# BloodAxe/segmentation-networks-benchmark

Hardware: AMD Instinct MI355X
Metric: images/sec/GPU (fwd+bwd) ZF_UNET 224x224 bs=32; 1/2/4/8-GPU scaling (higher is better)
Workload: dtype bf16; 1 GPU; ZF_UNET 224x224 bf16 bs=32/GPU, bce_dice, SGD lr 1e-3, Dropout2d 0.2, train step torch_train.py:180-190 (configs[1]); global_batch=32, parallelism=dp1

## Files before the change

segmentation-networks-benchmark_amd/csrc/common.h:

```cpp
#pragma once
#include <hip/hip_runtime.h>
#include <hip/hip_ext.h>
#include <stdint.h>
#include <stdio.h>
#include <string.h>

#include "../../include/segnb_hip.h"

typedef __attribute__((ext_vector_type(8))) __bf16 bf16x8_t;
typedef __attribute__((ext_vector_type(16))) float f32x16_t;

struct bf16_t {
    unsigned short bits;
};

void segnb_set_error(const char* fmt, ...);

#define SEGNB_CHECK_ARG(cond, msg)                                   \
    do {                                                             \
        if (!(cond)) {                                               \
            segnb_set_error("%s: bad argument: %s", __func__, msg);  \
            return SEGNB_E_BADARG;                                   \
        }                                                            \
    } while (0)
// ... 73 lines not shown
void segnb_plan_refuse(const char* why);
#define SEGNB_PLAN_REFUSE(why)                                         \
    SegnbPlanScope plan_scope__;                                       \
    if (plan_scope__.top && g_segnb_census_on) segnb_census(__func__); \
    if (plan_scope__.top && segnb_plan_recording()) segnb_plan_refuse(why)

int segnb_num_cus();
int segnb_knob_fprop_dma();
int segnb_knob_fprop_dma_cfg();
int segnb_knob_fprop_dma_dbg();
int segnb_knob_fprop_nostats();
int segnb_knob_rw_store_waves();
int segnb_knob_bnreduce_fused();
int segnb_knob_fprop_deepk();
int segnb_knob_fprop_thin();
enum segnb_try_outcome {
    SEGNB_TRY_DECLINED = 0,
    SEGNB_TRY_LAUNCHED,
    SEGNB_TRY_DELIVERED,
};
inline int segnb_try_launched(segnb_try_outcome* did, int rc) {
    if (rc == 0) *did = SEGNB_TRY_LAUNCHED;
    return rc;
}
int segnb_fprop_thin_try(segnb_try_outcome* did, const segnb_conv_geom* g, const void* in, const void* wpacked, void* out,
                         hipStream_t stream, const segnb_bn_reduce_epilogue* bn);
int segnb_fprop_thin_ok(const segnb_conv_geom* g);
int segnb_knob_fprop_upd();
int segnb_knob_fprop_drop();
int segnb_knob_fprop_mask();
int segnb_fprop_dma_actmask_ok(const segnb_conv_geom* g);
int segnb_fprop_roll_actmask_ok(const segnb_conv_geom* g);
int segnb_knob_fprop_mf16();
int segnb_knob_fprop_rw();
int segnb_knob_fprop_ksplit();
float* segnb_head_scratch(size_t bytes, hipStream_t stream);
void segnb_head_bwd_finish(const float* part, int gx, int gy, int K, int C, int CT, float* dw, float* db, hipStream_t stream);
int segnb_knob_pack_blocks();
int segnb_knob_fprop_roll();
int segnb_knob_wg_cu_pct();
int segnb_knob_conv_cus();
int segnb_fprop_dma_read_stamps(unsigned long long* host_dst);
int segnb_fprop_s1_try(segnb_try_outcome* did, const segnb_conv_geom* g, const void* in, const void* wpacked, const float* bias, int bias_n,
                       void* out, double* stats, hipStream_t stream, const float* drop = nullptr, int ld_drop = 0, int stats_ld = 0);
int segnb_fprop_dma_try(segnb_try_outcome* did, const segnb_conv_geom* g, const void* in, unsigned in_bytes, const void* wpacked,
                        unsigned w_bytes, const float* bias, int bias_n, void* out, double* stats,
                        hipStream_t stream, const segnb_act_epilogue* ep = nullptr, const segnb_upcat_src* uc = nullptr,
                        const segnb_bn_reduce_epilogue* bn = nullptr);
int segnb_fprop_rw_try(segnb_try_outcome* did, const segnb_conv_geom* g, const void* in, unsigned in_bytes, const void* wpacked,
                       unsigned w_bytes, const float* bias, int bias_n, void* out, double* stats,
                       hipStream_t stream, const segnb_bn_reduce_epilogue* bn = nullptr,
                       const segnb_act_epilogue* ep = nullptr, const segnb_upcat_src* uc = nullptr,
                       const segnb_upcat_src* upsum = nullptr);
int segnb_fprop_roll_try(segnb_try_outcome* did, const segnb_conv_geom* g, const void* in, unsigned in_bytes, const void* wpacked,
                         unsigned w_bytes, const float* bias, int bias_n, void* out, double* stats, hipStream_t stream,
                         const segnb_bn_reduce_epilogue* bn = nullptr, const segnb_operand_tf* tf = nullptr,
                         const segnb_upcat_src* uc = nullptr);
int segnb_fprop_c8_try(segnb_try_outcome* did, const segnb_conv_geom* g, const void* in, const void* wpacked, const float* bias, int bias_n,
                       void* out, double* stats, hipStream_t stream, const segnb_act_epilogue* ep = nullptr);
struct segnb_wgrad_bnapply {
    const void* g;
    int ld_g;
    const void* y;
    int ld_y;
    const float* coef;
    const float* bcoef;
// ... 106 lines not shown
```

segmentation-networks-benchmark_amd/csrc/runtime.hip:

```cpp
#include <stdarg.h>
#include <stdlib.h>

#include "common.h"

static thread_local char g_err[512] = "";

void segnb_set_error(const char* fmt, ...) {
    va_list ap;
    va_start(ap, fmt);
    vsnprintf(g_err, sizeof(g_err), fmt, ap);
    va_end(ap);
}

int segnb_num_cus() {
    static int cus = 0;
    if (cus > 0) return cus;
    int dev = 0;
    hipDeviceProp_t prop;
    if (hipGetDevice(&dev) != hipSuccess || hipGetDeviceProperties(&prop, dev) != hipSuccess) return 256;
    cus = prop.multiProcessorCount > 0 ? prop.multiProcessorCount : 256;
    return cus;
}

extern "C" const char* segnb_last_error(void) { return g_err; }
// ... 232 lines not shown
}
static int g_pack_blocks = 0;
int segnb_knob_pack_blocks() { return g_pack_blocks; }

static int g_wgrad_roll = 0;
int segnb_knob_wgrad_roll() { return g_wgrad_roll; }
static int g_wgrad_c8roll = 1;
int segnb_knob_wgrad_c8roll() { return g_wgrad_c8roll; }
static int g_conv_cu_pct = 100;
int segnb_knob_conv_cus() {
    const int n = segnb_num_cus() * g_conv_cu_pct / 100;
    return n < 1 ? 1 : n;
}
static int g_wg_cu_pct = 0;
int segnb_knob_wg_cu_pct() { return g_wg_cu_pct; }
static int g_fprop_deepk = -2;
int segnb_knob_fprop_deepk() {
    if (g_fprop_deepk == -2) {
        const char* e = getenv("SEGNB_FPROP_DEEPK");
        g_fprop_deepk = (e != nullptr && e[0] == '0') ? 0 : 1;
    }
    return g_fprop_deepk;
}
static int g_fprop_thin = 1;
int segnb_knob_fprop_thin() { return g_fprop_thin; }
static int g_fprop_mf16 = -2;
int segnb_knob_fprop_mf16() {
    if (g_fprop_mf16 == -2) {
        const char* e = getenv("SEGNB_FPROP_MF16");
        g_fprop_mf16 = (e != nullptr && e[0] == '0') ? 0 : 1;
    }
    return g_fprop_mf16;
}
static int g_fprop_upd = -2;
int segnb_knob_fprop_upd() {
    if (g_fprop_upd == -2) {
        const char* e = getenv("SEGNB_FPROP_UPD");
        g_fprop_upd = (e != nullptr && e[0] == '0') ? 0 : 1;
    }
    return g_fprop_upd;
}
static int g_fprop_mask = -2;
int segnb_knob_fprop_mask() {
    if (g_fprop_mask == -2) {
        const char* e = getenv("SEGNB_FPROP_MASK");
        g_fprop_mask = (e != nullptr && e[0] == '0') ? 0 : 1;
    }
    return g_fprop_mask;
}
static int g_fprop_drop = -2;
int segnb_knob_fprop_drop() {
    if (g_fprop_drop == -2) {
        const char* e = getenv("SEGNB_FPROP_DROP");
        g_fprop_drop = (e != nullptr && e[0] == '0') ? 0 : 1;
    }
    return g_fprop_drop;
}
static int g_fprop_nostats = 1;
int segnb_knob_fprop_nostats() { return g_fprop_nostats; }
static int g_rw_store_waves = 4;
int segnb_knob_rw_store_waves() { return g_rw_store_waves; }
static int g_bnreduce_fused = -2;
int segnb_knob_bnreduce_fused() {
    if (g_bnreduce_fused == -2) {
        const char* e = getenv("SEGNB_BNREDUCE_FUSED");
        g_bnreduce_fused = (e != nullptr && e[0] == '0') ? 0 : 1;
// ... 80 lines not shown
    }
    if (strcmp(key, "fprop_drop") == 0) {
        g_fprop_drop = value ? 1 : 0;
        return 0;
    }
    if (strcmp(key, "fprop_mask") == 0) {
        g_fprop_mask = value ? 1 : 0;
        return 0;
    }
    if (strcmp(key, "fprop_nostats") == 0) {
        g_fprop_nostats = value ? 1 : 0;
        return 0;
    }
    if (strcmp(key, "rw_store_waves") == 0) {
        g_rw_store_waves = value == 2 ? 2 : (value == 8 ? 8 : 4);
        return 0;
    }
    if (strcmp(key, "bnreduce_fused") == 0) {
        g_bnreduce_fused = value ? 1 : 0;
        return 0;
    }
    if (strcmp(key, "fprop_deepk") == 0) {
        g_fprop_deepk = value ? 1 : 0;
        return 0;
    }
    if (strcmp(key, "fprop_thin") == 0) {
        g_fprop_thin = value ? 1 : 0;
        return 0;
    }
    if (strcmp(key, "fprop_mf16") == 0) {
        g_fprop_mf16 = value ? 1 : 0;
        return 0;
    }
    if (strcmp(key, "call_census") == 0) {
        g_segnb_census_on = value ? 1 : 0;
        return 0;
    }
    if (strcmp(key, "fprop_ksplit") == 0) {
        g_fprop_ksplit = value < 0 ? 0 : value;
        return 0;
    }
    if (strcmp(key, "fprop_dma_dbg") == 0) {
        g_fprop_dma_dbg = value;
        return 0;
    }
    segnb_set_error("segnb_tune: unknown key '%s'", key);
    return SEGNB_E_BADARG;
}

extern "C" int segnb_debug_stamps(unsigned long long* host_dst) {
    SEGNB_CHECK_ARG(host_dst != nullptr, "NULL destination");
    return segnb_fprop_dma_read_stamps(host_dst);
}
```

segmentation-networks-benchmark_amd/csrc/wgrad_s1.hip:

```cpp
#include "common.h"

#include <cstdlib>
#include <type_traits>

namespace {

typedef __attribute__((ext_vector_type(4))) __bf16 bf16x4_t;
typedef __attribute__((address_space(3))) bf16x4_t* lds_bf16x4_ptr;

__device__ __forceinline__ bf16x8_t tr_frag(const unsigned char* p, int row4_bytes) {
    const bf16x4_t lo = __builtin_amdgcn_ds_read_tr16_b64_v4bf16((lds_bf16x4_ptr)(p));
    const bf16x4_t hi = __builtin_amdgcn_ds_read_tr16_b64_v4bf16((lds_bf16x4_ptr)(p + row4_bytes));
    return __builtin_shufflevector(lo, hi, 0, 1, 2, 3, 4, 5, 6, 7);
}

typedef __attribute__((address_space(3))) unsigned char* lds_u8_ptr;
__device__ __forceinline__ unsigned lds_addr(const void* p) { return (unsigned)(uintptr_t)(lds_u8_ptr)p; }

#define SEGNB_TR_READ2(lo, hi, addr, off0, off1)                                           \
    asm volatile("ds_read_b64_tr_b16 %0, %2 offset:%3\n\tds_read_b64_tr_b16 %1, %2 offset:%4" \
                 : "=&v"(lo), "=&v"(hi)                                                    \
                 : "v"(addr), "n"(off0), "n"(off1))
#define SEGNB_MFMA(acc, af, bf) \
    asm volatile("v_mfma_f32_32x32x16_bf16 %0, %1, %2, %0" : "+a"(acc) : "v"(af), "v"(bf))
#define SEGNB_MFMA_V(acc, af, bf) \
    asm volatile("v_mfma_f32_32x32x16_bf16 %0, %1, %2, %0" : "+v"(acc) : "v"(af), "v"(bf))
#define SEGNB_WAIT_LGKM(n) asm volatile("s_waitcnt lgkmcnt(%0)" ::"n"(n))

#ifndef SEGNB_WG_TS
#define SEGNB_WG_TS 1
#endif
#ifndef SEGNB_WG_WS_DB
#define SEGNB_WG_WS_DB 0
#endif
#ifndef SEGNB_WG_PACE
#define SEGNB_WG_PACE 0
#endif
#ifndef SEGNB_WG_TALL
#define SEGNB_WG_TALL 1
#endif
#ifndef SEGNB_WG_EXP
#define SEGNB_WG_EXP 0
#endif

struct WgS1Args {
    const bf16_t* x;
    const bf16_t* dy;
    float* dwp;
    int N, H, W;
    int Hi, Wi;
    int Ci, Co, ld_x, ld_dy;
    int dhmin, dwmin;
    int dh[9], dw[9];
    int HB, WB, IT;
    int TCI_TILES;
// ... 15 lines not shown
__device__ __forceinline__ void wg_tap(f32x16_t (&acc)[9], const bf16x4_t (&fa)[2], bf16x4_t (&fbc)[9][2],
                                       bf16x4_t (&fbn)[9][2], const unsigned (&vb)[9]) {
    SEGNB_WAIT_LGKM(WAITN);
    const bf16x8_t af = __builtin_shufflevector(fa[0], fa[1], 0, 1, 2, 3, 4, 5, 6, 7);
    const bf16x8_t bf = __builtin_shufflevector(fbc[T][0], fbc[T][1], 0, 1, 2, 3, 4, 5, 6, 7);
    SEGNB_MFMA(acc[T], af, bf);
    if constexpr (MORE) SEGNB_TR_READ2(fbn[T][0], fbn[T][1], vb[T], OB, OB + 4 * SXB);
}

template <int S0, int SPW, int KSPLIT, int SEGS, int WT, int XC, int SX, int SY, int MID, typename F>
__device__ __forceinline__ void wg_slabs(f32x16_t (&acc)[9], bf16x4_t (&fa)[2][2], bf16x4_t (&fb)[2][9][2],
                                         unsigned va, const unsigned (&vb)[9], F& mid) {
    if constexpr (S0 < SPW) {
        if constexpr (S0 == MID) mid();
        constexpr int cur = S0 & 1, nxt = cur ^ 1;
        constexpr bool more = S0 + 1 < SPW;
        constexpr int sn = (S0 + 1) * KSPLIT;
        constexpr int oa = ((sn / SEGS) * WT + (sn % SEGS) * 16) * SY;
        constexpr int ob = ((sn / SEGS) * XC + (sn % SEGS) * 16) * SX;
        if constexpr (more) SEGNB_TR_READ2(fa[nxt][0], fa[nxt][1], va, oa, oa + 4 * SY);
        wg_tap<0, 15, more, ob, SX>(acc, fa[cur], fb[cur], fb[nxt], vb);
        wg_tap<1, more ? 15 : 14, more, ob, SX>(acc, fa[cur], fb[cur], fb[nxt], vb);
        wg_tap<2, more ? 15 : 12, more, ob, SX>(acc, fa[cur], fb[cur], fb[nxt], vb);
        wg_tap<3, more ? 15 : 10, more, ob, SX>(acc, fa[cur], fb[cur], fb[nxt], vb);
        wg_tap<4, more ? 15 : 8, more, ob, SX>(acc, fa[cur], fb[cur], fb[nxt], vb);
        wg_tap<5, more ? 15 : 6, more, ob, SX>(acc, fa[cur], fb[cur], fb[nxt], vb);
        wg_tap<6, more ? 15 : 4, more, ob, SX>(acc, fa[cur], fb[cur], fb[nxt], vb);
        wg_tap<7, more ? 15 : 2, more, ob, SX>(acc, fa[cur], fb[cur], fb[nxt], vb);
        wg_tap<8, more ? 15 : 0, more, ob, SX>(acc, fa[cur], fb[cur], fb[nxt], vb);
        wg_slabs<S0 + 1, SPW, KSPLIT, SEGS, WT, XC, SX, SY, MID>(acc, fa, fb, va, vb, mid);
    }
}

constexpr int ts_c(int G, int u) { return (u + G) & 1; }
constexpr int ts_b(int G, int u) { return (u + G) >> 1; }
constexpr int ts_fa(int G, int c) { return c == G ? 0 : 2; }
constexpr int ts_fb(int b) { return b == 0 ? 1 : b + 2; }
constexpr int ts_k(int G, int u) {
    const int ka = ts_fa(G, ts_c(G, u)), kb = ts_fb(ts_b(G, u));
    return ka > kb ? ka : kb;
}
constexpr int ts_wait(int G, int u, bool more) {
    const int w = (6 - ts_k(G, u)) * 2 + (more ? 2 * (u < 7 ? u : 7) : 0);
    return w > 15 ? 15 : w;
}

template <int G, int J, int OA, int OB, int SX, int SY>
__device__ __forceinline__ void ts_request(bf16x4_t (&fan)[2][2], bf16x4_t (&fbn)[5][2], unsigned va,
                                           const unsigned (&vb)[5]) {
    if constexpr (J == 0) {
        SEGNB_TR_READ2(fan[G][0], fan[G][1], va, OA + 64 * G, OA + 64 * G + 4 * SY);
    } else if constexpr (J == 2) {
        SEGNB_TR_READ2(fan[1 - G][0], fan[1 - G][1], va, OA + 64 * (1 - G), OA + 64 * (1 - G) + 4 * SY);
    } else {
        constexpr int B = J == 1 ? 0 : J - 2;
        SEGNB_TR_READ2(fbn[B][0], fbn[B][1], vb[B], OB, OB + 4 * SX);
    }
}

template <int G, int U, bool MORE, int OA, int OB, int SX, int SY>
__device__ __forceinline__ void ts_units(f32x16_t (&acc)[9], bf16x4_t (&fac)[2][2], bf16x4_t (&fbc)[5][2],
                                         bf16x4_t (&fan)[2][2], bf16x4_t (&fbn)[5][2], unsigned va,
                                         const unsigned (&vb)[5]) {
    if constexpr (U < 9) {
        constexpr int C = ts_c(G, U), B = ts_b(G, U);
        SEGNB_WAIT_LGKM(ts_wait(G, U, MORE));
        const bf16x8_t af = __builtin_shufflevector(fac[C][0], fac[C][1], 0, 1, 2, 3, 4, 5, 6, 7);
        const bf16x8_t bf = __builtin_shufflevector(fbc[B][0], fbc[B][1], 0, 1, 2, 3, 4, 5, 6, 7);
        SEGNB_MFMA_V(acc[U], af, bf);
        if constexpr (MORE && U < 7) ts_request<G, U, OA, OB, SX, SY>(fan, fbn, va, vb);
        ts_units<G, U + 1, MORE, OA, OB, SX, SY>(acc, fac, fbc, fan, fbn, va, vb);
    }
}

template <int G, int J, int SX, int SY>
__device__ __forceinline__ void ts_first(bf16x4_t (&fa0)[2][2], bf16x4_t (&fb0)[5][2], unsigned va,
                                         const unsigned (&vb)[5]) {
    if constexpr (J < 7) {
        ts_request<G, J, 0, 0, SX, SY>(fa0, fb0, va, vb);
        ts_first<G, J + 1, SX, SY>(fa0, fb0, va, vb);
    }
}

template <int G, int S0, int SPW, int SEGS, int WT, int XC, int SX, int SY, int MID, typename F>
__device__ __forceinline__ void ts_slabs(f32x16_t (&acc)[9], bf16x4_t (&fa)[2][2][2], bf16x4_t (&fb)[2][5][2],
                                         unsigned va, const unsigned (&vb)[5], F& mid) {
    if constexpr (S0 < SPW) {
        if constexpr (S0 == MID) mid();
        constexpr int cur = S0 & 1, nxt = cur ^ 1;
        constexpr bool more = S0 + 1 < SPW;
        constexpr int sn = S0 + 1;
        constexpr int oa = ((sn / SEGS) * WT + (sn % SEGS) * 16) * SY;
        constexpr int ob = ((sn / SEGS) * XC + (sn % SEGS) * 16) * SX;
        ts_units<G, 0, more, oa, ob, SX, SY>(acc, fa[cur], fb[cur], fa[nxt], fb[nxt], va, vb);
        ts_slabs<G, S0 + 1, SPW, SEGS, WT, XC, SX, SY, MID>(acc, fa, fb, va, vb, mid);
    }
}

template <int G, int SPW, int SEGS, int WT, int XC, int SX, int SY, int MID, typename F>
__device__ __forceinline__ void ts_iteration(f32x16_t (&acc)[9], unsigned va, const unsigned (&vb)[5], F& mid) {
    bf16x4_t fa[2][2][2], fb[2][5][2];
    ts_first<G, 0, SX, SY>(fa[0], fb[0], va, vb);
    ts_slabs<G, 0, SPW, SEGS, WT, XC, SX, SY, MID>(acc, fa, fb, va, vb, mid);
}

template <int T, int SXB>
__device__ __forceinline__ void wg_first(bf16x4_t (&fb0)[9][2], const unsigned (&vb)[9]) {
    if constexpr (T < 9) {
        SEGNB_TR_READ2(fb0[T][0], fb0[T][1], vb[T], 0, 4 * SXB);
        wg_first<T + 1, SXB>(fb0, vb);
    }
}

constexpr bool wg_double_buffered(int tile_bytes) { return 2 * tile_bytes <= 160 * 1024; }

constexpr int lds_stride(int channels) {
    int s = channels * 2;
    while (!((s % 256) == 64 || (s % 256) == 192)) s += 16;
    return s;
}

template <int R, int WT, bool FLAT>
struct WgTile {
    static constexpr int W2 = WT + 2;
    static constexpr int PD = FLAT ? (WT * W2 + 15) / 16 * 16 : R * WT;
    static constexpr int XT = FLAT ? PD + 2 * W2 + 2 : (R + 2) * (WT + 2);
    static constexpr int XROWS = FLAT ? R * XT : XT, YROWS = FLAT ? R * PD : PD;
    static constexpr int NSLAB = YROWS / 16;
    static constexpr int SEGS = FLAT ? PD / 16 : WT / 16;
    static constexpr int YSTEP = FLAT ? PD : WT, XSTEP = FLAT ? XT : WT + 2;
};

template <int BCO, int BCI, int R, int WT, bool FLAT>
constexpr bool wg_specialised() {
    using TL = WgTile<R, WT, FLAT>;
    return SEGNB_WG_TS && BCO == 64 && BCI == 64;
}
template <int BCO, int BCI, int R, int WT, bool FLAT>
constexpr bool wg_ws_db() {
    using TL = WgTile<R, WT, FLAT>;
    return SEGNB_WG_WS_DB && wg_specialised<BCO, BCI, R, WT, FLAT>() &&
           wg_double_buffered(TL::XROWS * lds_stride(BCI) + TL::YROWS * lds_stride(BCO));
}

template <int BCO, int BCI, int R, int WT, bool FLAT = false, bool BNA = false>
__global__ __launch_bounds__((wg_specialised<BCO, BCI, R, WT, FLAT>() ? 512 : 256), 1) void conv_wgrad_s1x9_kernel(
    const WgS1Args a) {
    static_assert(!BNA || (!FLAT && BCO == 32), "the recomputed dy operand is built for the thin 32 x 32 tiles");
    using TL = WgTile<R, WT, FLAT>;
    constexpr int TCO = BCO / 32, TCI = BCI / 32;
    constexpr int NSUB = TCO * TCI;
    static_assert(NSUB == 1 || NSUB == 4, "tile is 32x32 or 64x64");
    constexpr int KSPLIT = 4 / NSUB;
    constexpr int XC = FLAT ? TL::W2 : WT + 2;
    constexpr int SX = lds_stride(BCI), SY = lds_stride(BCO);
    constexpr int NSLAB = TL::NSLAB;
    constexpr int SEGS = TL::SEGS;
    constexpr int XCH = TL::XROWS * (BCI / 8);
    constexpr int YCH = TL::YROWS * (BCO / 8);
    constexpr int XPT = (XCH + 255) / 256, YPT = (YCH + 255) / 256;

    constexpr int BUF = TL::XROWS * SX + TL::YROWS * SY;
    constexpr bool DB = wg_ws_db<BCO, BCI, R, WT, FLAT>();

// ... 49 lines not shown
        if constexpr (FLAT) {
#pragma unroll
            for (int u = 0; u < XPT; ++u) {
                const int c = tid + u * 256;
                const int row = c / (BCI / 8), cc = c - row * (BCI / 8);
                const int g = row / TL::XT, q = row - g * TL::XT;
                const int n = it * R + g;
                const int hi = q / TL::W2 + a.dhmin, wi = q % TL::W2 + a.dwmin;
                const int ch = ci0 + cc * 8;
                uint4 v = make_uint4(0, 0, 0, 0);
                if (c < XCH && n < a.N && ch < a.Ci && (unsigned)hi < (unsigned)a.Hi && (unsigned)wi < (unsigned)a.Wi) {
                    if (a.u != nullptr && ch < a.Cu)
                        v = *reinterpret_cast<const uint4*>(a.u + ((long long)(n * (a.Hi >> 1) + (hi >> 1)) * (a.Wi >> 1) + (wi >> 1)) * a.ld_u + ch);
                    else
                        v = *reinterpret_cast<const uint4*>(a.x + ((long long)(n * a.Hi + hi) * a.Wi + wi) * a.ld_x + (ch - (a.u != nullptr ? a.Cu : 0)));
                }
                rx[u] = v;
            }
#pragma unroll
            for (int u = 0; u < YPT; ++u) {
                const int c = tid + u * 256;
                const int row = c / (BCO / 8), cc = c - row * (BCO / 8);
                const int g = row / TL::PD, pp = row - g * TL::PD;
                const int n = it * R + g;
                const int ho = pp / TL::W2, wo = pp % TL::W2;
                const int ch = co0 + cc * 8;
                uint4 v = make_uint4(0, 0, 0, 0);
                if (c < YCH && n < a.N && ch < a.Co && ho < a.H && wo < a.W)
                    v = *reinterpret_cast<const uint4*>(a.dy + ((long long)(n * a.H + ho) * a.W + wo) * a.ld_dy + ch);
                ry[u] = v;
            }
            return;
        }
        const int n = it / (a.HB * a.WB);
        const int rem = it - n * (a.HB * a.WB);
        const int hb = rem / a.WB, wb = rem - hb * a.WB;
        const int h0 = hb * R, w0 = wb * WT;
#pragma unroll
        for (int u = 0; u < XPT; ++u) {
            const int c = tid + u * 256;
            const int pix = c / (BCI / 8), cc = c - pix * (BCI / 8);
            const int xr = pix / XC, xc = pix - xr * XC;
            const int hi = h0 + a.dhmin + xr, wi = w0 + a.dwmin + xc;
            const int ch = ci0 + cc * 8;
            uint4 v = make_uint4(0, 0, 0, 0);
            if (c < XCH && ch < a.Ci && (unsigned)hi < (unsigned)a.Hi && (unsigned)wi < (unsigned)a.Wi) {
                if (a.u != nullptr && ch < a.Cu)
                    v = *reinterpret_cast<const uint4*>(a.u + ((long long)(n * (a.Hi >> 1) + (hi >> 1)) * (a.Wi >> 1) + (wi >> 1)) * a.ld_u + ch);
                else
                    v = *reinterpret_cast<const uint4*>(a.x + ((long long)(n * a.Hi + hi) * a.Wi + wi) * a.ld_x + (ch - (a.u != nullptr ? a.Cu : 0)));
            }
            rx[u] = v;
        }
#pragma unroll
        for (int u = 0; u < YPT; ++u) {
            const int c = tid + u * 256;
            const int pix = c / (BCO / 8), cc = c - pix * (BCO / 8);
            const int yr = pix / WT, yc = pix - yr * WT;
            const int ho = h0 + yr, wo = w0 + yc;
            const int ch = co0 + cc * 8;
            uint4 v = make_uint4(0, 0, 0, 0);
            if (c < YCH && ch < a.Co && ho < a.H && wo < a.W) {
                if constexpr (BNA) {
                    const long long pix = (long long)(n * a.H + ho) * a.W + wo;
                    float gv[8], yv[8], o[8];
                    load8(reinterpret_cast<const bf16_t*>(a.bna.g) + pix * a.bna.ld_g + ch, gv);
// ... 15 lines not shown
            ry[u] = v;
        }
    };
    auto gload = [&](int it) { gload_to(it, rx, ry); };
    auto lstore_from = [&](int bo, auto paced, const auto& rx, const auto& ry) {
        constexpr bool PACED = decltype(paced)::value;
#pragma unroll
        for (int u = 0; u < XPT; ++u) {
            const int c = tid + u * 256;
            if (c < XCH) {
                const int pix = c / (BCI / 8), cc = c - pix * (BCI / 8);
                *reinterpret_cast<uint4*>(sX + bo + pix * SX + cc * 16) = rx[u];
            }
            if constexpr (PACED && SEGNB_WG_PACE > 0) __builtin_amdgcn_s_sleep(SEGNB_WG_PACE);
        }
#pragma unroll
        for (int u = 0; u < YPT; ++u) {
            const int c = tid + u * 256;
            if (c < YCH) {
                const int pix = c / (BCO / 8), cc = c - pix * (BCO / 8);
                *reinterpret_cast<uint4*>(sY + bo + pix * SY + cc * 16) = ry[u];
            }
            if constexpr (PACED && SEGNB_WG_PACE > 0) __builtin_amdgcn_s_sleep(SEGNB_WG_PACE);
        }
    };
    auto lstore = [&](int bo, auto paced) { lstore_from(bo, paced, rx, ry); };
    constexpr std::false_type burst{};
    constexpr std::true_type paced{};

    const int tg = TS ? __builtin_amdgcn_readfirstlane(wave >> 1) : 0;
    const int sub = TS ? 0 : wave / KSPLIT, kpart = TS ? 0 : wave - sub * KSPLIT;
    const int sco = TS ? 0 : sub / TCI, sci = TS ? (wave & 1) : sub - sco * TCI;
    const int q = (lane & 15) >> 2, p = lane & 3, h = lane >> 5, cbase = 16 * ((lane >> 4) & 1);
    const int a_off = (8 * h + q) * SY + (sco * 32 + cbase + 4 * p) * 2;
    const int b_off = (8 * h + q) * SX + (sci * 32 + cbase + 4 * p) * 2;
    int tap_off[9];
#pragma unroll
    for (int t = 0; t < 9; ++t) tap_off[t] = (a.dh[t] * XC + a.dw[t]) * SX;

    if constexpr (TS) {
        if (fetcher) {
            gload(it_begin);
            lstore(0, burst);
            if constexpr (DB) {
                if (it_begin + 1 < it_end) gload_to(it_begin + 1, rx, ry);
                if (it_begin + 2 < it_end) gload_to(it_begin + 2, rx2, ry2);
                __syncthreads();
                int cur = 0;
                for (int it = it_begin; it < it_end; it += 2) {
                    if (it + 1 < it_end) lstore_from((cur ^ 1) * BUF, paced, rx, ry);
                    if (it + 3 < it_end) gload_to(it + 3, rx, ry);
                    __syncthreads();
                    if (it + 1 >= it_end) break;
                    if (it + 2 < it_end) lstore_from(cur * BUF, paced, rx2, ry2);
                    if (it + 4 < it_end) gload_to(it + 4, rx2, ry2);
                    __syncthreads();
                }
                return;
            }
            __syncthreads();
            for (int it = it_begin; it < it_end; ++it) {
#if !(SEGNB_WG_EXP & 1)
                if (it + 1 < it_end) gload(it + 1);
#endif
                __syncthreads();
                if (it + 1 < it_end) {
// ... 25 lines not shown
    __syncthreads();
    constexpr int SPW = NSLAB / KSPLIT;
    static_assert(KSPLIT == 1 || KSPLIT % SEGS == 0, "slab -> (row, segment) split");
    const int krow = kpart / SEGS, kseg = kpart - krow * SEGS;
    const unsigned va = lds_addr(sY + a_off) + (unsigned)((krow * TL::YSTEP + kseg * 16) * SY);
    unsigned vb[9];
#pragma unroll
    for (int t = 0; t < 9; ++t) vb[t] = lds_addr(sX + b_off + tap_off[t]) + (unsigned)((krow * TL::XSTEP + kseg * 16) * SX);
    auto pixel_loop = [&](auto Gc) {
        constexpr int G = decltype(Gc)::value;
        if constexpr (DB) {
            int cur = 0;
            for (int it = it_begin; it < it_end; ++it) {
                const bool more = it + 1 < it_end;
                if constexpr (!TS) {
                    if (more) gload(it + 1);
                }
                const unsigned bo = (unsigned)(cur * BUF);
                const unsigned vac = va + bo;
                auto mid = [&]() {
                    if constexpr (!TS) {
                        if (more) lstore((cur ^ 1) * BUF, burst);
                    }
                };
#if SEGNB_WG_EXP & 2
                mid();
                if (false) {
#else
                if constexpr (TS) {
#endif
                    unsigned vtc[5];
#pragma unroll
                    for (int b = 0; b < 5; ++b) vtc[b] = vb[4 * G + b] + bo;
                    ts_iteration<G, SPW, SEGS, TL::YSTEP, TL::XSTEP, SX, SY, (SPW + 1) / 2>(acc, vac, vtc, mid);
                } else if constexpr (!(SEGNB_WG_EXP & 2)) {
                    unsigned vbc[9];
#pragma unroll
                    for (int t = 0; t < 9; ++t) vbc[t] = vb[t] + bo;
                    bf16x4_t fa[2][2], fb[2][9][2];
                    SEGNB_TR_READ2(fa[0][0], fa[0][1], vac, 0, 4 * SY);
                    wg_first<0, SX>(fb[0], vbc);
                    wg_slabs<0, SPW, KSPLIT, SEGS, TL::YSTEP, TL::XSTEP, SX, SY, (SPW + 1) / 2>(acc, fa, fb, vac, vbc,
                                                                                                mid);
                }
                __syncthreads();
                cur ^= 1;
            }
            asm volatile("s_nop 7\n\ts_nop 7\n\ts_nop 7" ::);
        } else {
            auto mid = [] {};
            for (int it = it_begin; it < it_end; ++it) {
                if constexpr (!TS) {
                    if (it + 1 < it_end) gload(it + 1);
                }
                if constexpr (TS) {
#if !(SEGNB_WG_EXP & 2)
                    unsigned vtc[5];
#pragma unroll
                    for (int b = 0; b < 5; ++b) vtc[b] = vb[4 * G + b];
                    ts_iteration<G, SPW, SEGS, TL::YSTEP, TL::XSTEP, SX, SY, -1>(acc, va, vtc, mid);
#endif
                } else {
                    bf16x4_t fa[2][2], fb[2][9][2];
                    SEGNB_TR_READ2(fa[0][0], fa[0][1], va, 0, 4 * SY);
                    wg_first<0, SX>(fb[0], vb);
                    wg_slabs<0, SPW, KSPLIT, SEGS, TL::YSTEP, TL::XSTEP, SX, SY, -1>(acc, fa, fb, va, vb, mid);
                }
                asm volatile("s_nop 7\n\ts_nop 7\n\ts_nop 7" ::);
                __syncthreads();
                if (it + 1 < it_end) {
                    if constexpr (!TS) lstore(0, burst);
                    __syncthreads();
                }
            }
        }
    };
    if (TS && tg != 0)
        pixel_loop(std::integral_constant<int, 1>{});
    else
        pixel_loop(std::integral_constant<int, 0>{});

    if (KSPLIT > 1) {
        float* sAcc = reinterpret_cast<float*>(smem);
        for (int w = 1; w < KSPLIT; ++w) {
            if (wave == w) {
#pragma unroll
                for (int t = 0; t < 9; ++t)
#pragma unroll
                    for (int e = 0; e < 16; ++e) {
                        float* dst = sAcc + (t * 16 + e) * 64 + lane;
                        *dst = (w == 1) ? acc[t][e] : (*dst + acc[t][e]);
                    }
            }
// ... 311 lines not shown

int s1_slabs(int tiles, bool thin, bool flat = false) {
    static const double frac_wide = [] {
        const char* e = getenv("SEGNB_WG_CU_FRACTION");
        const double r = e ? atof(e) : 0.5;
        return r <= 0.0 ? 1.0 : r;
    }();
    static const double frac_thin = [] {
        const char* e = getenv("SEGNB_WG_CU_FRACTION_THIN");
        const double r = e ? atof(e) : 1.0;
        return r <= 0.0 ? 1.0 : r;
    }();
    constexpr double frac_flat = -1.0;
    const int pct = segnb_knob_wg_cu_pct();
    const double wide = pct > 0 ? pct / 100.0 : frac_wide;
    const double frac = thin ? frac_thin : ((flat && frac_flat > 0.0) ? frac_flat : wide);
    int S = (int)(segnb_num_cus() * frac) / tiles;
    return S < 1 ? 1 : S;
}

template <int BCO, int BCI, int R, int WT, bool FLAT = false, bool BNA = false>
int launch_s1(WgS1Args& a, int nslab, hipStream_t stream, bool partial, const segnb_wgrad_target* tgt = nullptr) {
    using TL = WgTile<R, WT, FLAT>;
    constexpr int tile_bytes = TL::XROWS * lds_stride(BCI) + TL::YROWS * lds_stride(BCO);
    constexpr int smem = wg_ws_db<BCO, BCI, R, WT, FLAT>() ? 2 * tile_bytes : tile_bytes;
    static_assert(smem <= 160 * 1024, "tiles fit the LDS");
    static int attr_rc = [] {
        hipError_t e = hipFuncSetAttribute(reinterpret_cast<const void*>(conv_wgrad_s1x9_kernel<BCO, BCI, R, WT, FLAT, BNA>),
                                           hipFuncAttributeMaxDynamicSharedMemorySize, smem);
        if (e != hipSuccess) segnb_set_error("wgrad_s1 hipFuncSetAttribute: %s", hipGetErrorString(e));
        return (int)e;
    }();
    if (attr_rc) return attr_rc;
    a.HB = (a.H + R - 1) / R;
    a.WB = (a.W + WT - 1) / WT;
    a.IT = FLAT ? (a.N + R - 1) / R : a.N * a.HB * a.WB;
    const int ncot = (a.Co + BCO - 1) / BCO;
    a.TCI_TILES = (a.Ci + BCI - 1) / BCI;
    const int tiles = ncot * a.TCI_TILES;
    const int S = s1_slabs(tiles, BCO == 32, FLAT);
    if (S != nslab) {
        segnb_set_error("segnb_conv_wgrad: workspace has %d slabs, this geometry needs %d (segnb_conv_wgrad_slabs)",
                        nslab, S);
        return SEGNB_E_BADARG;
    }
    a.its_per_split = (a.IT + S - 1) / S;
    a.slab_stride = (long long)a.Co * a.Ktot;
    a.gw = nullptr;
    if (tgt != nullptr && S == 1) {
        a.gw = tgt->gw;
        a.gw_s_out = tgt->s_out;
        a.gw_s_in = tgt->s_in; a.gw_ci_off = tgt->ci_off; a.gw_Ci = tgt->Ci; a.gw_Co = tgt->Co; a.gw_acc = tgt->accumulate;
        for (int t = 0; t < 9; ++t) a.gw_kpos[t] = tgt->kpos[t];
    }
    hipLaunchKernelGGL((conv_wgrad_s1x9_kernel<BCO, BCI, R, WT, FLAT, BNA>), dim3(tiles * S),
                       dim3(wg_specialised<BCO, BCI, R, WT, FLAT>() ? 512 : 256), smem, stream, a);
    if (S > 1 && !partial) {
        const long long total = a.slab_stride;
        if (S <= 16 && total % 4 == 0)
            hipLaunchKernelGGL(slab_reduce_few_kernel, dim3((unsigned)((total / 4 + 255) / 256)), dim3(256), 0, stream,
                               reinterpret_cast<float4*>(a.dwp), total / 4, S);
        else
            hipLaunchKernelGGL(slab_reduce_kernel, dim3((unsigned)((total + 63) / 64)), dim3(256), 0, stream, a.dwp,
                               total, S);
    }
    return 0;
}

struct S1Choice {
    int cfg;
    int bco, bci;
};
S1Choice s1_choose(const segnb_conv_geom* g) {
    S1Choice c = {0, 0, 0};
    if (g->ntaps != 9 || g->in_step != 1 || g->out_step != 1 || g->oh0 != 0 || g->ow0 != 0) return c;
    if (g->QH != g->Ho || g->QW != g->Wo) return c;
    int dhmin = g->dh[0], dhmax = g->dh[0], dwmin = g->dw[0], dwmax = g->dw[0];
    for (int t = 1; t < 9; ++t) {
        dhmin = g->dh[t] < dhmin ? g->dh[t] : dhmin;
        dhmax = g->dh[t] > dhmax ? g->dh[t] : dhmax;
        dwmin = g->dw[t] < dwmin ? g->dw[t] : dwmin;
        dwmax = g->dw[t] > dwmax ? g->dw[t] : dwmax;
    }
    if (dhmax - dhmin != 2 || dwmax - dwmin != 2) return c;
    const bool thin = g->Co <= 32 || g->Ci <= 32;
    if (thin) {
        if (g->Wo < 24) return c;
        c = {(g->Ho % 16 == 0 && g->Ho >= 64 && SEGNB_WG_TALL) ? 6 : 1, 32, 32};
    } else if (g->Wo > 16) {
        constexpr int rows = 8;
        constexpr bool w16 = true;
        if (w16 && g->Wo % 16 == 0 && g->Wo % 32 != 0)
            c = {3, 64, 64};
        else
            c = {(rows == 8 && g->Ho % 8 == 0) ? 7 : ((rows >= 7 && g->Ho % 7 == 0) ? 8 : 2), 64, 64};
    } else if (g->Wo == 14 && g->Ho == 14) {
        c = {5, 64, 64};
    } else if (g->Wo >= 12) {
        c = {3, 64, 64};
    } else if (g->Wo == 7 && g->Ho == 7) {
        c = {4, 64, 64};
    }
    return c;
}


struct WgSxArgs {
    const bf16_t* x;
    const bf16_t* dy;
    float* dwp;
    int N, H, W, Hi, Wi;
    int Ci, Co, ld_x, ld_dy;
    int dhmin, dwmin;
    int ntaps;
    int HB, WB, IT, TCI_TILES, its_per_split;
    long long slab_stride;
    int Ktot;
    signed char dh[SEGNB_MAX_TAPS], dw[SEGNB_MAX_TAPS];
};

constexpr int lds_stride_step(int channels, int step) {
// ... 283 lines not shown
    if (bna != nullptr && c.cfg != 1 && c.cfg != 6) return 0;
    int dhmin = g->dh[0], dwmin = g->dw[0];
    for (int t = 1; t < 9; ++t) {
        dhmin = g->dh[t] < dhmin ? g->dh[t] : dhmin;
        dwmin = g->dw[t] < dwmin ? g->dw[t] : dwmin;
    }
    WgS1Args a;
    a.x = (const bf16_t*)in;
    a.dy = (const bf16_t*)dout;
    a.dwp = dwp;
    a.N = g->N; a.H = g->Ho; a.W = g->Wo; a.Hi = g->Hi; a.Wi = g->Wi;
    a.Ci = g->Ci; a.Co = g->Co; a.ld_x = g->ld_in; a.ld_dy = g->ld_out;
    a.dhmin = dhmin; a.dwmin = dwmin;
    for (int t = 0; t < 9; ++t) {
        a.dh[t] = g->dh[t] - dhmin;
        a.dw[t] = g->dw[t] - dwmin;
    }
    a.Ktot = 9 * g->Ci;
    a.u = uc != nullptr ? (const bf16_t*)uc->u : nullptr;
    a.Cu = uc != nullptr ? uc->Cu : 0;
    a.ld_u = uc != nullptr ? uc->ld_u : 0;
    a.bna = segnb_wgrad_bnapply{};
    int rc;
    if (bna != nullptr) {
        a.bna = *bna;
        rc = c.cfg == 1 ? launch_s1<32, 32, 8, 32, false, true>(a, nslab, stream, partial, tgt)
                        : launch_s1<32, 32, 16, 32, false, true>(a, nslab, stream, partial, tgt);
    } else if (c.cfg == 1) rc = launch_s1<32, 32, 8, 32>(a, nslab, stream, partial, tgt);
    else if (c.cfg == 6) rc = launch_s1<32, 32, 16, 32>(a, nslab, stream, partial, tgt);
    else if (c.cfg == 2) rc = launch_s1<64, 64, 4, 32>(a, nslab, stream, partial, tgt);
    else if (c.cfg == 7) rc = launch_s1<64, 64, 8, 32>(a, nslab, stream, partial, tgt);
    else if (c.cfg == 8) rc = launch_s1<64, 64, 7, 32>(a, nslab, stream, partial, tgt);
    else if (c.cfg == 3) rc = launch_s1<64, 64, 8, 16>(a, nslab, stream, partial, tgt);
    else if (c.cfg == 4) rc = launch_s1<64, 64, 4, 7, true>(a, nslab, stream, partial, tgt);
    else rc = launch_s1<64, 64, 1, 14, true>(a, nslab, stream, partial, tgt);
    if (rc) return rc;
    *did = tgt != nullptr && nslab == 1 ? SEGNB_TRY_DELIVERED : SEGNB_TRY_LAUNCHED;
    return 0;
}


int segnb_wgrad_sx_slabs(const segnb_conv_geom* g) {
    const SxChoice c = sx_choose(g);
    if (!c.cfg) return 0;
    return s1_slabs(((g->Co + c.bco - 1) / c.bco) * ((g->Ci + c.bci - 1) / c.bci), true);
}

int segnb_wgrad_sx_try(segnb_try_outcome* did, const segnb_conv_geom* g, const void* in, const void* dout, float* dwp, int nslab,
                       hipStream_t stream, bool partial) {
    *did = SEGNB_TRY_DECLINED;
    const SxChoice c = sx_choose(g);
    if (!c.cfg) return 0;
    int dhmin = g->dh[0], dwmin = g->dw[0];
    for (int t = 1; t < g->ntaps; ++t) {
        dhmin = g->dh[t] < dhmin ? g->dh[t] : dhmin;
        dwmin = g->dw[t] < dwmin ? g->dw[t] : dwmin;
    }
    WgSxArgs a;
    a.x = (const bf16_t*)in;
    a.dy = (const bf16_t*)dout;
    a.dwp = dwp;
    a.N = g->N; a.H = g->Ho; a.W = g->Wo; a.Hi = g->Hi; a.Wi = g->Wi;
    a.Ci = g->Ci; a.Co = g->Co; a.ld_x = g->ld_in; a.ld_dy = g->ld_out;
    a.dhmin = dhmin; a.dwmin = dwmin;
    a.ntaps = g->ntaps;
    for (int t = 0; t < g->ntaps; ++t) {
// ... 23 lines not shown
```

Before: 6838 images/s.

## Add dense full-width row tiles for stride-1 wgrad at widths 56 and 28

```diff
diff --git a/segmentation-networks-benchmark_amd/csrc/common.h b/segmentation-networks-benchmark_amd/csrc/common.h
--- a/segmentation-networks-benchmark_amd/csrc/common.h
+++ b/segmentation-networks-benchmark_amd/csrc/common.h
@@ -129,6 +129,7 @@
 int segnb_fprop_dma_actmask_ok(const segnb_conv_geom* g);
 int segnb_fprop_roll_actmask_ok(const segnb_conv_geom* g);
 int segnb_knob_fprop_mf16();
+int segnb_knob_wgrad_dense();
 int segnb_knob_fprop_rw();
 int segnb_knob_fprop_ksplit();
 float* segnb_head_scratch(size_t bytes, hipStream_t stream);
diff --git a/segmentation-networks-benchmark_amd/csrc/runtime.hip b/segmentation-networks-benchmark_amd/csrc/runtime.hip
--- a/segmentation-networks-benchmark_amd/csrc/runtime.hip
+++ b/segmentation-networks-benchmark_amd/csrc/runtime.hip
@@ -288,6 +288,14 @@
     }
     return g_fprop_mf16;
 }
+static int g_wgrad_dense = -2;
+int segnb_knob_wgrad_dense() {
+    if (g_wgrad_dense == -2) {
+        const char* e = getenv("SEGNB_WGRAD_DENSE");
+        g_wgrad_dense = e != nullptr && e[0] >= '0' && e[0] <= '2' ? e[0] - '0' : 1;
+    }
+    return g_wgrad_dense;
+}
 static int g_fprop_upd = -2;
 int segnb_knob_fprop_upd() {
     if (g_fprop_upd == -2) {
@@ -434,6 +442,10 @@
         g_fprop_mf16 = value ? 1 : 0;
         return 0;
     }
+    if (strcmp(key, "wgrad_dense") == 0) {
+        g_wgrad_dense = value < 0 ? 0 : (value > 2 ? 2 : value);
+        return 0;
+    }
     if (strcmp(key, "call_census") == 0) {
         g_segnb_census_on = value ? 1 : 0;
         return 0;
diff --git a/segmentation-networks-benchmark_amd/csrc/wgrad_s1.hip b/segmentation-networks-benchmark_amd/csrc/wgrad_s1.hip
--- a/segmentation-networks-benchmark_amd/csrc/wgrad_s1.hip
+++ b/segmentation-networks-benchmark_amd/csrc/wgrad_s1.hip
@@ -21,6 +21,14 @@
     asm volatile("ds_read_b64_tr_b16 %0, %2 offset:%3\n\tds_read_b64_tr_b16 %1, %2 offset:%4" \
                  : "=&v"(lo), "=&v"(hi)                                                    \
                  : "v"(addr), "n"(off0), "n"(off1))
+#define SEGNB_TR_READ2_C(lo, hi, addr, clo, chi, off0, off1)                                                   \
+    do {                                                                                                        \
+        unsigned t0_, t1_;                                                                                      \
+        asm volatile("v_add_u32 %2, %4, %5\n\tv_add_u32 %3, %4, %6\n\t"                                         \
+                     "ds_read_b64_tr_b16 %0, %2 offset:%7\n\tds_read_b64_tr_b16 %1, %3 offset:%8"                   \
+                     : "=&v"(lo), "=&v"(hi), "=&v"(t0_), "=&v"(t1_)                                             \
+                     : "v"(addr), "v"(clo), "v"(chi), "n"(off0), "n"(off1));                                   \
+    } while (0)
 #define SEGNB_MFMA(acc, af, bf) \
     asm volatile("v_mfma_f32_32x32x16_bf16 %0, %1, %2, %0" : "+a"(acc) : "v"(af), "v"(bf))
 #define SEGNB_MFMA_V(acc, af, bf) \
@@ -102,6 +110,34 @@
     }
 }
 
+template <int R, int WT, bool FLAT>
+struct WgTile {
+    static constexpr bool DENSE = !FLAT && WT % 16 != 0;
+    static constexpr int RP = DENSE ? 4 : R, P = R / RP;
+    static_assert(!DENSE || (R % RP == 0 && RP * WT % 16 == 0 && WT > 16), "dense tiles: whole slabs per panel, one row end per slab");
+    static constexpr int W2 = WT + 2;
+    static constexpr int PD = FLAT ? (WT * W2 + 15) / 16 * 16 : R * WT;
+    static constexpr int XT = FLAT ? PD + 2 * W2 + 2 : P * (RP + 2) * (WT + 2);
+    static constexpr int XROWS = FLAT ? R * XT : XT, YROWS = FLAT ? R * PD : PD;
+    static constexpr int NSLAB = YROWS / 16;
+    static constexpr int SEGS = FLAT ? PD / 16 : (DENSE ? 1 : WT / 16);
+    static constexpr int YSTEP = FLAT ? PD : WT, XSTEP = FLAT ? XT : WT + 2;
+};
+
+template <typename TL>
+constexpr int wg_ya(int s) {
+    return TL::DENSE ? 16 * s : ((s / TL::SEGS) * TL::YSTEP + (s % TL::SEGS) * 16);
+}
+template <typename TL>
+constexpr int wg_xb(int s) {
+    return TL::DENSE ? 16 * s + 2 * (16 * s / TL::YSTEP) + 2 * (16 * s / (TL::RP * TL::YSTEP)) * TL::XSTEP
+                     : ((s / TL::SEGS) * TL::XSTEP + (s % TL::SEGS) * 16);
+}
+template <typename TL>
+constexpr int wg_xcross(int s) {
+    return TL::DENSE && (16 * s) % TL::YSTEP + 15 >= TL::YSTEP ? (16 * s) % TL::YSTEP : 0;
+}
+
 constexpr int ts_c(int G, int u) { return (u + G) & 1; }
 constexpr int ts_b(int G, int u) { return (u + G) >> 1; }
 constexpr int ts_fa(int G, int c) { return c == G ? 0 : 2; }
@@ -115,63 +151,66 @@
     return w > 15 ? 15 : w;
 }
 
-template <int G, int J, int OA, int OB, int SX, int SY>
+template <int G, int J, int SN, typename TL, int SX, int SY>
 __device__ __forceinline__ void ts_request(bf16x4_t (&fan)[2][2], bf16x4_t (&fbn)[5][2], unsigned va,
-                                           const unsigned (&vb)[5]) {
+                                           const unsigned (&vb)[5], int rl) {
+    constexpr int OA = wg_ya<TL>(SN) * SY, OB = wg_xb<TL>(SN) * SX, XM = wg_xcross<TL>(SN);
     if constexpr (J == 0) {
         SEGNB_TR_READ2(fan[G][0], fan[G][1], va, OA + 64 * G, OA + 64 * G + 4 * SY);
     } else if constexpr (J == 2) {
         SEGNB_TR_READ2(fan[1 - G][0], fan[1 - G][1], va, OA + 64 * (1 - G), OA + 64 * (1 - G) + 4 * SY);
     } else {
         constexpr int B = J == 1 ? 0 : J - 2;
-        SEGNB_TR_READ2(fbn[B][0], fbn[B][1], vb[B], OB, OB + 4 * SX);
-    }
-}
-
-template <int G, int U, bool MORE, int OA, int OB, int SX, int SY>
+        if constexpr (XM == 0) {
+            SEGNB_TR_READ2(fbn[B][0], fbn[B][1], vb[B], OB, OB + 4 * SX);
+        } else {
+            const unsigned clo = rl >= TL::YSTEP - XM ? 2u * SX : 0u, chi = rl + 4 >= TL::YSTEP - XM ? 2u * SX : 0u;
+            SEGNB_TR_READ2_C(fbn[B][0], fbn[B][1], vb[B], clo, chi, OB, OB + 4 * SX);
+        }
+    }
+}
+
+template <int G, int U, bool MORE, int SN, typename TL, int SX, int SY>
 __device__ __forceinline__ void ts_units(f32x16_t (&acc)[9], bf16x4_t (&fac)[2][2], bf16x4_t (&fbc)[5][2],
                                          bf16x4_t (&fan)[2][2], bf16x4_t (&fbn)[5][2], unsigned va,
-                                         const unsigned (&vb)[5]) {
+                                         const unsigned (&vb)[5], int rl) {
     if constexpr (U < 9) {
         constexpr int C = ts_c(G, U), B = ts_b(G, U);
         SEGNB_WAIT_LGKM(ts_wait(G, U, MORE));
         const bf16x8_t af = __builtin_shufflevector(fac[C][0], fac[C][1], 0, 1, 2, 3, 4, 5, 6, 7);
         const bf16x8_t bf = __builtin_shufflevector(fbc[B][0], fbc[B][1], 0, 1, 2, 3, 4, 5, 6, 7);
         SEGNB_MFMA_V(acc[U], af, bf);
-        if constexpr (MORE && U < 7) ts_request<G, U, OA, OB, SX, SY>(fan, fbn, va, vb);
-        ts_units<G, U + 1, MORE, OA, OB, SX, SY>(acc, fac, fbc, fan, fbn, va, vb);
-    }
-}
-
-template <int G, int J, int SX, int SY>
+        if constexpr (MORE && U < 7) ts_request<G, U, SN, TL, SX, SY>(fan, fbn, va, vb, rl);
+        ts_units<G, U + 1, MORE, SN, TL, SX, SY>(acc, fac, fbc, fan, fbn, va, vb, rl);
+    }
+}
+
+template <int G, int J, typename TL, int SX, int SY>
 __device__ __forceinline__ void ts_first(bf16x4_t (&fa0)[2][2], bf16x4_t (&fb0)[5][2], unsigned va,
-                                         const unsigned (&vb)[5]) {
+                                         const unsigned (&vb)[5], int rl) {
     if constexpr (J < 7) {
-        ts_request<G, J, 0, 0, SX, SY>(fa0, fb0, va, vb);
-        ts_first<G, J + 1, SX, SY>(fa0, fb0, va, vb);
-    }
-}
-
-template <int G, int S0, int SPW, int SEGS, int WT, int XC, int SX, int SY, int MID, typename F>
+        ts_request<G, J, 0, TL, SX, SY>(fa0, fb0, va, vb, rl);
+        ts_first<G, J + 1, TL, SX, SY>(fa0, fb0, va, vb, rl);
+    }
+}
+
+template <int G, int S0, int SPW, typename TL, int SX, int SY, int MID, typename F>
 __device__ __forceinline__ void ts_slabs(f32x16_t (&acc)[9], bf16x4_t (&fa)[2][2][2], bf16x4_t (&fb)[2][5][2],
-                                         unsigned va, const unsigned (&vb)[5], F& mid) {
+                                         unsigned va, const unsigned (&vb)[5], int rl, F& mid) {
     if constexpr (S0 < SPW) {
         if constexpr (S0 == MID) mid();
         constexpr int cur = S0 & 1, nxt = cur ^ 1;
         constexpr bool more = S0 + 1 < SPW;
-        constexpr int sn = S0 + 1;
-        constexpr int oa = ((sn / SEGS) * WT + (sn % SEGS) * 16) * SY;
-        constexpr int ob = ((sn / SEGS) * XC + (sn % SEGS) * 16) * SX;
-        ts_units<G, 0, more, oa, ob, SX, SY>(acc, fa[cur], fb[cur], fa[nxt], fb[nxt], va, vb);
-        ts_slabs<G, S0 + 1, SPW, SEGS, WT, XC, SX, SY, MID>(acc, fa, fb, va, vb, mid);
-    }
-}
-
-template <int G, int SPW, int SEGS, int WT, int XC, int SX, int SY, int MID, typename F>
-__device__ __forceinline__ void ts_iteration(f32x16_t (&acc)[9], unsigned va, const unsigned (&vb)[5], F& mid) {
+        ts_units<G, 0, more, S0 + 1, TL, SX, SY>(acc, fa[cur], fb[cur], fa[nxt], fb[nxt], va, vb, rl);
+        ts_slabs<G, S0 + 1, SPW, TL, SX, SY, MID>(acc, fa, fb, va, vb, rl, mid);
+    }
+}
+
+template <int G, int SPW, typename TL, int SX, int SY, int MID, typename F>
+__device__ __forceinline__ void ts_iteration(f32x16_t (&acc)[9], unsigned va, const unsigned (&vb)[5], int rl, F& mid) {
     bf16x4_t fa[2][2][2], fb[2][5][2];
-    ts_first<G, 0, SX, SY>(fa[0], fb[0], va, vb);
-    ts_slabs<G, 0, SPW, SEGS, WT, XC, SX, SY, MID>(acc, fa, fb, va, vb, mid);
+    ts_first<G, 0, TL, SX, SY>(fa[0], fb[0], va, vb, rl);
+    ts_slabs<G, 0, SPW, TL, SX, SY, MID>(acc, fa, fb, va, vb, rl, mid);
 }
 
 template <int T, int SXB>
@@ -189,17 +228,6 @@
     while (!((s % 256) == 64 || (s % 256) == 192)) s += 16;
     return s;
 }
-
-template <int R, int WT, bool FLAT>
-struct WgTile {
-    static constexpr int W2 = WT + 2;
-    static constexpr int PD = FLAT ? (WT * W2 + 15) / 16 * 16 : R * WT;
-    static constexpr int XT = FLAT ? PD + 2 * W2 + 2 : (R + 2) * (WT + 2);
-    static constexpr int XROWS = FLAT ? R * XT : XT, YROWS = FLAT ? R * PD : PD;
-    static constexpr int NSLAB = YROWS / 16;
-    static constexpr int SEGS = FLAT ? PD / 16 : WT / 16;
-    static constexpr int YSTEP = FLAT ? PD : WT, XSTEP = FLAT ? XT : WT + 2;
-};
 
 template <int BCO, int BCI, int R, int WT, bool FLAT>
 constexpr bool wg_specialised() {
@@ -315,6 +343,41 @@
             }
             return;
         }
+        if constexpr (TL::DENSE) {
+#pragma unroll
+            for (int u = 0; u < XPT; ++u) {
+                const int c = tid + u * 256;
+                const int pix = c / (BCI / 8), cc = c - pix * (BCI / 8);
+                const int xr = pix / XC, xc = pix - xr * XC;
+                const int k = xr / (TL::RP + 2), lr = xr - k * (TL::RP + 2);
+                const int qb = it * TL::P + k, n = qb / a.HB;
+                const int hi = (qb - n * a.HB) * TL::RP + a.dhmin + lr, wi = a.dwmin + xc;
+                const int ch = ci0 + cc * 8;
+                uint4 v = make_uint4(0, 0, 0, 0);
+                if (c < XCH && n < a.N && ch < a.Ci && (unsigned)hi < (unsigned)a.Hi && (unsigned)wi < (unsigned)a.Wi) {
+                    if (a.u != nullptr && ch < a.Cu)
+                        v = *reinterpret_cast<const uint4*>(a.u + ((long long)(n * (a.Hi >> 1) + (hi >> 1)) * (a.Wi >> 1) + (wi >> 1)) * a.ld_u + ch);
+                    else
+                        v = *reinterpret_cast<const uint4*>(a.x + ((long long)(n * a.Hi + hi) * a.Wi + wi) * a.ld_x + (ch - (a.u != nullptr ? a.Cu : 0)));
+                }
+                rx[u] = v;
+            }
+#pragma unroll
+            for (int u = 0; u < YPT; ++u) {
+                const int c = tid + u * 256;
+                const int pix = c / (BCO / 8), cc = c - pix * (BCO / 8);
+                const int yr = pix / WT, wo = pix - yr * WT;
+                const int k = yr / TL::RP, lr = yr - k * TL::RP;
+                const int qb = it * TL::P + k, n = qb / a.HB;
+                const int ho = (qb - n * a.HB) * TL::RP + lr;
+                const int ch = co0 + cc * 8;
+                uint4 v = make_uint4(0, 0, 0, 0);
+                if (c < YCH && n < a.N && ch < a.Co && ho < a.H && wo < a.W)
+                    v = *reinterpret_cast<const uint4*>(a.dy + ((long long)(n * a.H + ho) * a.W + wo) * a.ld_dy + ch);
+                ry[u] = v;
+            }
+            return;
+        }
         const int n = it / (a.HB * a.WB);
         const int rem = it - n * (a.HB * a.WB);
         const int hb = rem / a.WB, wb = rem - hb * a.WB;
@@ -396,6 +459,7 @@
     const int sub = TS ? 0 : wave / KSPLIT, kpart = TS ? 0 : wave - sub * KSPLIT;
     const int sco = TS ? 0 : sub / TCI, sci = TS ? (wave & 1) : sub - sco * TCI;
     const int q = (lane & 15) >> 2, p = lane & 3, h = lane >> 5, cbase = 16 * ((lane >> 4) & 1);
+    const int rl = 8 * h + q;
     const int a_off = (8 * h + q) * SY + (sco * 32 + cbase + 4 * p) * 2;
     const int b_off = (8 * h + q) * SX + (sci * 32 + cbase + 4 * p) * 2;
     int tap_off[9];
@@ -487,7 +551,7 @@
                     unsigned vtc[5];
 #pragma unroll
                     for (int b = 0; b < 5; ++b) vtc[b] = vb[4 * G + b] + bo;
-                    ts_iteration<G, SPW, SEGS, TL::YSTEP, TL::XSTEP, SX, SY, (SPW + 1) / 2>(acc, vac, vtc, mid);
+                    ts_iteration<G, SPW, TL, SX, SY, (SPW + 1) / 2>(acc, vac, vtc, rl, mid);
                 } else if constexpr (!(SEGNB_WG_EXP & 2)) {
                     unsigned vbc[9];
 #pragma unroll
@@ -513,7 +577,7 @@
                     unsigned vtc[5];
 #pragma unroll
                     for (int b = 0; b < 5; ++b) vtc[b] = vb[4 * G + b];
-                    ts_iteration<G, SPW, SEGS, TL::YSTEP, TL::XSTEP, SX, SY, -1>(acc, va, vtc, mid);
+                    ts_iteration<G, SPW, TL, SX, SY, -1>(acc, va, vtc, rl, mid);
 #endif
                 } else {
                     bf16x4_t fa[2][2], fb[2][9][2];
@@ -891,9 +955,13 @@
         return (int)e;
     }();
     if (attr_rc) return attr_rc;
-    a.HB = (a.H + R - 1) / R;
+    a.HB = (a.H + TL::RP - 1) / TL::RP;
     a.WB = (a.W + WT - 1) / WT;
-    a.IT = FLAT ? (a.N + R - 1) / R : a.N * a.HB * a.WB;
+    a.IT = FLAT ? (a.N + R - 1) / R : (TL::DENSE ? (a.N * a.HB + TL::P - 1) / TL::P : a.N * a.HB * a.WB);
+    if (TL::DENSE && a.W != WT) {
+        segnb_set_error("wgrad_s1: dense tiles of %d columns for an image %d wide", WT, a.W);
+        return SEGNB_E_BADARG;
+    }
     const int ncot = (a.Co + BCO - 1) / BCO;
     a.TCI_TILES = (a.Ci + BCI - 1) / BCI;
     const int tiles = ncot * a.TCI_TILES;
@@ -946,6 +1014,8 @@
     if (thin) {
         if (g->Wo < 24) return c;
         c = {(g->Ho % 16 == 0 && g->Ho >= 64 && SEGNB_WG_TALL) ? 6 : 1, 32, 32};
+    } else if ((segnb_knob_wgrad_dense() >= 1 && g->Wo == 56) || (segnb_knob_wgrad_dense() >= 2 && g->Wo == 28)) {
+        c = {g->Wo == 56 ? 9 : 10, 64, 64};
     } else if (g->Wo > 16) {
         constexpr int rows = 8;
         constexpr bool w16 = true;
@@ -1295,6 +1365,8 @@
     else if (c.cfg == 7) rc = launch_s1<64, 64, 8, 32>(a, nslab, stream, partial, tgt);
     else if (c.cfg == 8) rc = launch_s1<64, 64, 7, 32>(a, nslab, stream, partial, tgt);
     else if (c.cfg == 3) rc = launch_s1<64, 64, 8, 16>(a, nslab, stream, partial, tgt);
+    else if (c.cfg == 9) rc = launch_s1<64, 64, 4, 56>(a, nslab, stream, partial, tgt);
+    else if (c.cfg == 10) rc = launch_s1<64, 64, 8, 28>(a, nslab, stream, partial, tgt);
     else if (c.cfg == 4) rc = launch_s1<64, 64, 4, 7, true>(a, nslab, stream, partial, tgt);
     else rc = launch_s1<64, 64, 1, 14, true>(a, nslab, stream, partial, tgt);
     if (rc) return rc;
```

Result: no change. 6846 images/s (median of 6 runs) (+0.1%).
